# furio1999/EO_Diffusion

Hardware: AMD Instinct MI355X
Metric: denoising steps/sec (UNet fwd + DDPM update) at 256x256 bs=16 (higher is better)
Workload: dtype f32; 1 GPU; DDPM sampling step, 256x256x3, batch 16 per GPU, UNet arch A0 (base 128, mults [1,2,3,4], 1 res-block(s), attn_res []), Philox noise, x0-clipped update; global_batch=16, image_size=256, parallelism=batch-sharded x1, accumulate=fp32, precision_mode=fp32x3

## Files before the change

### eo_diffusion_amd/csrc/igemm.hip

```cpp
#include <type_traits>

#include "common.h"

struct IgemmP {
    const char* a0;
    const char* a1;
    const char* b;
    const float* bias;
    const float* cbias;
    const char* res;
    char* y;
    long long cbias_stride;
    int N, H, W, C0, C1, Cin, Cout, KS, stride, pad, ups, pad_tl, Ho, Wo, HoWo, Heff, Weff;
    int tw_log2, th;
    int tiles_pw, tiles_pi;
    long long lda, ldb, ldc, sa0, sa1, sb0, sb1, sc0, sc1;
    int nb1, bias_mode, c_f32;
    long long M;
    int Ncols, K, taps, KT, tiles_m, tiles_n, out_nchw;
    int kc0, kc1;
    int tapmajor_log2;
    int ldk;
    const float* gn_ss;
    int gn_silu;
// ... 1021 lines not shown
            const int hi = (UPS ? tg.ty0 / 2 : tg.ty0) - 1 + py, wi = (UPS ? tg.tx0 / 2 : tg.tx0) - 1 + px;
            const bool ok = (wave + NW * i) < PG && prow < PR && (unsigned)hi < (unsigned)p.H && (unsigned)wi < (unsigned)p.W;
            if (ok) pvalid |= 1u << i;
            ppix[i] = (unsigned)(hi * p.W + wi);
        }
    };
    set_tile_pieces(g);
    auto pchunk_of = [&](int i) { return (int)((pck >> (3 * i)) & 7u); };
    unsigned b_v[LB];
#pragma unroll
    for (int i = 0; i < LB; ++i) {
        const int row = (wave + NW * i) * 8 + srow;
        b_v[i] = (n0 + row < p.Ncols) ? (unsigned)(row * p.Cin * ES) + bchunk0 * 16 : EOD_OOB;
    }
    const __amdgpu_buffer_rsrc_t rsA0 = make_rsrc(p.a0 + (long long)g.n_first * p.H * p.W * p.C0 * ES);
    const __amdgpu_buffer_rsrc_t rsA1 = make_rsrc(p.a1 ? p.a1 + (long long)g.n_first * p.H * p.W * p.C1 * ES : p.a0);
    const __amdgpu_buffer_rsrc_t rsB = make_rsrc(p.b + (long long)n0 * p.Cin * ES);
    const int tapstride = p.Cout * p.Cin * ES;
    __amdgpu_buffer_rsrc_t rsS = rsB;
    if constexpr (GN)
        rsS = __builtin_amdgcn_make_buffer_rsrc(const_cast<float*>(p.gn_ss) + (long long)g.n_first * p.Cin * 2, 0, p.Cin * 8, 0x00020000);

    struct Chunk {
        int src, kin, cw;
        unsigned bk;
        bool ktail;
    };
    auto chunk_of = [&](int cc) {
        Chunk c;
        c.src = cc >= p.kc0 ? 1 : 0;
        const int ci = c.src ? cc - p.kc0 : cc;
        c.kin = ci * BK;
        c.cw = c.src ? p.C1 : p.C0;
        c.bk = (unsigned)(((c.src ? p.C0 : 0) + c.kin) * ES);
        c.ktail = c.kin + BK > c.cw;
        return c;
    };
    auto issue_patch_piece = [&](int i, const Chunk& c, char* abuf) {
        const int pc = pchunk_of(i);
        unsigned v = ((pvalid >> i) & 1u) ? ppix[i] * (unsigned)(c.cw * ES) + pc * 16 : EOD_OOB;
        if (__builtin_expect(c.ktail, 0)) v = (c.kin + pc * EPC < c.cw) ? v : EOD_OOB;
        if (c.src)
            blds16(rsA1, v, (unsigned)(c.kin * ES), abuf + (wave + NW * i) * 1024);
        else
            blds16(rsA0, v, (unsigned)(c.kin * ES), abuf + (wave + NW * i) * 1024);
    };
    auto issue_ss = [&](const Chunk& c, char* ssbuf) {
        const unsigned v = lane < 32 ? (unsigned)(lane * 16 + ((c.src ? p.C0 : 0) + c.kin) * 8) : EOD_OOB;
        __builtin_amdgcn_raw_ptr_buffer_load_lds(rsS, (lds_void*)ssbuf, 16, v, 0, 0, 0);
    };
    struct XfPre {
        i32x4 raw;
        f32x4 q[GN ? (ES == 2 ? 4 : 2) : 1];
    };
    auto xf_load = [&](int i, char* abuf, const char* ssbuf, XfPre& pre) {
        const int pc = pchunk_of(i);
        pre.raw = *reinterpret_cast<const i32x4*>(abuf + (wave + NW * i) * 1024 + lane * 16);
        if constexpr (GN) {
            const float* sp = reinterpret_cast<const float*>(ssbuf) + pc * EPC * 2;
#pragma unroll
            for (int k = 0; k < (ES == 2 ? 4 : 2); ++k) pre.q[k] = *reinterpret_cast<const f32x4*>(sp + 4 * k);
        }
    };
    auto xf_finish = [&](int i, const Chunk& c, char* abuf, const XfPre& pre) {
        const int pc = pchunk_of(i);
        const bool ok = ((pvalid >> i) & 1u) && (!c.ktail || (c.kin + pc * EPC < c.cw));
        char* ptr = abuf + (wave + NW * i) * 1024 + lane * 16;
        const i32x4 raw = pre.raw;
        i32x4 outv = raw;
        if constexpr (GN) {
            if constexpr (ES == 2) {
                const half8 h = __builtin_bit_cast(half8, raw);
                half8 o;
#pragma unroll
                for (int e = 0; e < 8; ++e) {
                    float v = (float)h[e] * pre.q[e >> 1][(e & 1) * 2] + pre.q[e >> 1][(e & 1) * 2 + 1];
                    v = v * __builtin_amdgcn_rcpf(1.0f + __builtin_amdgcn_exp2f(__builtin_fmaf(v, silu_k, silu_c)));
                    o[e] = (half_t)v;
                }
                outv = __builtin_bit_cast(i32x4, o);
            } else {
                const f32x4 f = __builtin_bit_cast(f32x4, raw);
                f32x4 o;
                const f32x4 q0 = pre.q[0], q1 = pre.q[GN && ES != 2 ? 1 : 0];
                const float sc[4] = {q0[0], q0[2], q1[0], q1[2]}, sh[4] = {q0[1], q0[3], q1[1], q1[3]};
#pragma unroll
                for (int e = 0; e < 4; ++e) {
                    float v = f[e] * sc[e] + sh[e];
                    if constexpr (SPLIT) {
                        v = v * __builtin_amdgcn_rcpf(1.0f + __builtin_amdgcn_exp2f(__builtin_fmaf(v, silu_k, silu_c)));
                    } else {
                        if (p.gn_silu) v = silu_f<SPLIT>(v);
                    }
                    o[e] = v;
                }
                outv = __builtin_bit_cast(i32x4, o);
            }
            if constexpr (!SPLIT) {
                if (!ok) outv = raw;
            }
        }
        if constexpr (SPLIT) {
            const float sl = (GN && !ok) ? 0.0f : asc.s;
            *reinterpret_cast<i32x4*>(ptr) = split_pair_exchange_scaled(__builtin_bit_cast(f32x4, outv), sl, (pc & 1) != 0);
        } else {
            if (ok) *reinterpret_cast<i32x4*>(ptr) = outv;
        }
    };
    auto transform_piece = [&](int i, const Chunk& c, char* abuf, const char* ssbuf) {
        XfPre pre;
        xf_load(i, abuf, ssbuf, pre);
        xf_finish(i, c, abuf, pre);
    };
    unsigned bve[LB];
    auto weight_offsets = [&](const Chunk& c, unsigned (&out)[LB]) {
        const bool kok = !c.ktail || (c.kin + (SPLIT ? (bchunk0 >> 1) * 8 : bchunk0 * EPC) < c.cw);
#pragma unroll
        for (int i = 0; i < LB; ++i) out[i] = kok ? b_v[i] : EOD_OOB;
    };
    auto issue_weights_at = [&](int tap, const Chunk& c, const unsigned (&off)[LB], char* bst) {
        const unsigned soff = (unsigned)(tap * tapstride) + c.bk;
#pragma unroll
        for (int i = 0; i < LB; ++i) blds16(rsB, off[i], soff, bst + (wave + NW * i) * 1024);
    };
    auto issue_weights = [&](int tap, const Chunk& c, char* bst) {
        unsigned off[LB];
        weight_offsets(c, off);
        issue_weights_at(tap, c, off, bst);
    };

    typename AccLayout<MS>::vec acc[TM][TN];
#pragma unroll
    for (int i = 0; i < TM; ++i)
#pragma unroll
        for (int j = 0; j < TN; ++j)
#pragma unroll
            for (int r = 0; r < AccLayout<MS>::R; ++r) acc[i][j][r] = 0.0f;

    const int lr = lane & (MS - 1), lh = MS == 32 ? lane >> 5 : lane >> 4;
    int prow0[TM], pyo[TM], pxo[TM];
#pragma unroll
    for (int i = 0; i < TM; ++i) {
        const int r = wm * WM + i * MS + lr;
        pyo[i] = r >> 4;
        pxo[i] = r & 15;
        prow0[i] = pyo[i] * PW + pxo[i];
    }
    const int bsw = (lr >> 1) & 7;
    int bcoff[4];
#pragma unroll
    for (int s = 0; s < 4; ++s) bcoff[s] = ((2 * s + lh) ^ bsw) * 16;
    const int b_rd = (wn * WN + lr) * BKB;
    int acur[2][3] = {{0, 0, 0}, {0, 0, 0}};
    auto aimm = [](int i, int dy) { return (UPS ? ((i + dy + 1) >> 1) : (i + dy)) * PW * BKB; };
    if constexpr (MS == 16) {
        constexpr int LROW = WM / 16;
        static_assert(LROW % 2 == 0, "the UPS row split needs an even first tile row per wave");
        const int c0 = SPLIT ? 2 * ((0x2130 >> (4 * lh)) & 3) : lh, c1 = SPLIT ? c0 + 1 : 4 + lh;
#pragma unroll
        for (int dx = 0; dx < 3; ++dx) {
            const int pxc = UPS ? ((lr + dx + 1) >> 1) : lr + dx;
            const int key = (pxc >> 1) & 7;
            const int rowb = ((UPS ? (wm * LROW) >> 1 : wm * LROW) * PW + pxc) * BKB;
            acur[0][dx] = rowb + ((c0 ^ key) << 4);
            acur[1][dx] = rowb + ((c1 ^ key) << 4);
        }
    }

    const int KC = p.kc0 + p.kc1;
    int kc_begin = 0, kc_end = KC;
    if constexpr (KSPLIT) {
        kc_begin = (int)blockIdx.y * p.splitk_per;
        kc_end = (int)blockIdx.y == p.splitk - 1 ? KC : kc_begin + p.splitk_per;
    }
    const int NSTEP = (kc_end - kc_begin) * 9;
    const int TSTEP = NSTEP * ntile;
    {
        const Chunk c0 = chunk_of(kc_begin);
#pragma unroll
        for (int i = 0; i < LAH; ++i)
            if ((wave + NW * i) < PG) issue_patch_piece(i, c0, sA);
        if constexpr (GN) {
            if (wave == 0) issue_ss(c0, sS);
        }
        issue_weights(0, c0, sB);
        if constexpr (XF) {
            asm volatile("s_waitcnt vmcnt(0)" ::: "memory");
            if constexpr (GN) __builtin_amdgcn_s_barrier();
#pragma unroll
            for (int i = 0; i < LAH; ++i)
                if ((wave + NW * i) < PG) transform_piece(i, c0, sA, sS);
            __builtin_amdgcn_s_waitcnt(0xc07f);
        }
    }
    EOD_STAMP_AT(1);
    int pp1 = 0;
    int step = 0;
    int qpar = 0;
    for (int k = 0; k < ntile; ++k) {
    for (int cc = kc_begin; cc < kc_end; ++cc) {
        const Chunk cur = chunk_of(cc);
        const bool next_tile = STREAM && cc + 1 == kc_end && k + 1 < ntile;
        const bool has_next = cc + 1 < kc_end || next_tile;
        const Chunk nxt = chunk_of(cc + 1 < kc_end ? cc + 1 : (next_tile ? 0 : cc));
        if constexpr (STREAM) {
            if (next_tile) set_tile_pieces(make_geom<true, BM>(p, tile_m + k + 1));
        }
        const char* abuf = sA + qpar * ABUF;
        char* abuf_next = sA + (qpar ^ 1) * ABUF;
        weight_offsets(cur, bve);
#pragma unroll
        for (int t = 0; t < 9; ++t, ++step) {
            EOD_TSTAMP_AT(4 * t + 0);
            if (!(STREAM && t == 0 && cc == kc_begin && k > 0)) {
                if (pp1 == 0) asm volatile("s_waitcnt vmcnt(0)" ::: "memory");
                else if (pp1 == 1) asm volatile("s_waitcnt vmcnt(1)" ::: "memory");
                else asm volatile("s_waitcnt vmcnt(2)" ::: "memory");
                if constexpr (XF) __builtin_amdgcn_s_waitcnt(0xc07f);
                __builtin_amdgcn_s_barrier();
            }
            EOD_TSTAMP_AT(4 * t + 1);
            if (step + 1 < TSTEP) {
                if (t < 8) issue_weights_at(t + 1, cur, bve, sB + ((step + 1) & 1) * BSTAGE);
                else issue_weights(0, nxt, sB + ((step + 1) & 1) * BSTAGE);
            }
            pp1 = 0;
            if (t < LAH && has_next && (wave + NW * t) < PG) {
                issue_patch_piece(t, nxt, abuf_next);
                pp1 = 1;
            }
            if constexpr (GN) {
                if (t == 0 && has_next && wave == 0) {
                    issue_ss(nxt, sS + (qpar ^ 1) * 1024);
                    ++pp1;
                }
            }
            EOD_TSTAMP_AT(4 * t + 2);
            const int dy = t / 3, dx = t - dy * 3;
            const char* bst = sB + (step & 1) * BSTAGE;
            int arow[TM], asw[TM];
#pragma unroll
            for (int i = 0; i < TM; ++i) {
                const int pxc = UPS ? ((pxo[i] + dx + 1) >> 1) : pxo[i] + dx;
                const int prow = UPS ? ((pyo[i] + dy + 1) >> 1) * PW + pxc : prow0[i] + dy * PW + dx;
                arow[i] = prow * BKB;
                asw[i] = (pxc >> 1) & 7;
            }
            if constexpr (MS == 16 && SPLIT) {
                const int ch = 2 * ((0x2130 >> (4 * lh)) & 3);
                i32x4 ah[TM], al[TM], bh[TN], bl[TN];
#pragma unroll
                for (int i = 0; i < TM; ++i) al[i] = *reinterpret_cast<const i32x4*>(sA + acur[1][dx] + aimm(i, dy));
#pragma unroll
                for (int j = 0; j < TN; ++j) bh[j] = *reinterpret_cast<const i32x4*>(bst + b_rd + j * MS * BKB + ((ch ^ bsw) << 4));
#pragma unroll
                for (int i = 0; i < TM; ++i) ah[i] = *reinterpret_cast<const i32x4*>(sA + acur[0][dx] + aimm(i, dy));
#pragma unroll
                for (int i = 0; i < TM; ++i)
#pragma unroll
                    for (int j = 0; j < TN; ++j)
                        acc[i][j] = DIRECT ? __builtin_amdgcn_mfma_f32_16x16x32_f16(__builtin_bit_cast(half8, bh[j]), __builtin_bit_cast(half8, al[i]), acc[i][j], 0, 0, 0)
                                           : __builtin_amdgcn_mfma_f32_16x16x32_f16(__builtin_bit_cast(half8, al[i]), __builtin_bit_cast(half8, bh[j]), acc[i][j], 0, 0, 0);
#pragma unroll
                for (int j = 0; j < TN; ++j) bl[j] = *reinterpret_cast<const i32x4*>(bst + b_rd + j * MS * BKB + (((ch + 1) ^ bsw) << 4));
#pragma unroll
                for (int i = 0; i < TM; ++i)
#pragma unroll
                    for (int j = 0; j < TN; ++j)
                        acc[i][j] = DIRECT ? __builtin_amdgcn_mfma_f32_16x16x32_f16(__builtin_bit_cast(half8, bl[j]), __builtin_bit_cast(half8, ah[i]), acc[i][j], 0, 0, 0)
                                           : __builtin_amdgcn_mfma_f32_16x16x32_f16(__builtin_bit_cast(half8, ah[i]), __builtin_bit_cast(half8, bl[j]), acc[i][j], 0, 0, 0);
#pragma unroll
                for (int i = 0; i < TM; ++i)
#pragma unroll
                    for (int j = 0; j < TN; ++j)
                        acc[i][j] = DIRECT ? __builtin_amdgcn_mfma_f32_16x16x32_f16(__builtin_bit_cast(half8, bh[j]), __builtin_bit_cast(half8, ah[i]), acc[i][j], 0, 0, 0)
                                           : __builtin_amdgcn_mfma_f32_16x16x32_f16(__builtin_bit_cast(half8, ah[i]), __builtin_bit_cast(half8, bh[j]), acc[i][j], 0, 0, 0);
            } else if constexpr (MS == 16) {
#pragma unroll
                for (int s = 0; s < 2; ++s) {
                    const int ch = 4 * s + lh;
                    i32x4 fa16[TM], fb16[TN];
#pragma unroll
                    for (int i = 0; i < TM; ++i) fa16[i] = *reinterpret_cast<const i32x4*>(sA + acur[s][dx] + aimm(i, dy));
#pragma unroll
                    for (int j = 0; j < TN; ++j) fb16[j] = *reinterpret_cast<const i32x4*>(bst + b_rd + j * MS * BKB + ((ch ^ bsw) << 4));
#pragma unroll
                    for (int i = 0; i < TM; ++i)
#pragma unroll
                        for (int j = 0; j < TN; ++j)
                            acc[i][j] = __builtin_amdgcn_mfma_f32_16x16x32_f16(__builtin_bit_cast(half8, fa16[i]), __builtin_bit_cast(half8, fb16[j]), acc[i][j], 0, 0, 0);
                }
            } else {
            i32x4 fa[2][TM], fb[2][TN];
#pragma unroll
            for (int i = 0; i < TM; ++i)
                fa[0][i] = *reinterpret_cast<const i32x4*>(abuf + arow[i] + (((0 + lh) ^ asw[i]) << 4));
#pragma unroll
            for (int j = 0; j < TN; ++j) fb[0][j] = *reinterpret_cast<const i32x4*>(bst + b_rd + j * 32 * BKB + bcoff[0]);
            __builtin_amdgcn_sched_group_barrier(0x100, TM + TN, 0);
#pragma unroll
            for (int s = 0; s < 4; ++s) {
                const int cur = s & 1, nx = cur ^ 1;
                if (s < 3) {
#pragma unroll
                    for (int i = 0; i < TM; ++i)
                        fa[nx][i] = *reinterpret_cast<const i32x4*>(abuf + arow[i] + (((2 * (s + 1) + lh) ^ asw[i]) << 4));
#pragma unroll
                    for (int j = 0; j < TN; ++j)
                        fb[nx][j] = *reinterpret_cast<const i32x4*>(bst + b_rd + j * 32 * BKB + bcoff[s + 1]);
                    __builtin_amdgcn_sched_group_barrier(0x100, TM + TN, 0);
                }
#pragma unroll
                for (int i = 0; i < TM; ++i)
#pragma unroll
                    for (int j = 0; j < TN; ++j) Mma<T>::run(fa[cur][i], fb[cur][j], acc[i][j]);
                __builtin_amdgcn_sched_group_barrier(0x008, TM * TN * (sizeof(T) == 4 ? 4 : 1), 0);
            }
            }
            EOD_TSTAMP_AT(4 * t + 3);
            if constexpr (XF) {
                if (t >= 2 && t - 2 < LAH && has_next && (wave + NW * (t - 2)) < PG)
                    transform_piece(t - 2, nxt, abuf_next, sS + (qpar ^ 1) * 1024);
            }
        }
        EOD_TSTAMP_AT(36);
#ifdef EOD_TSTAMP
        if (GN && wave == 1 && cc == 1 && k == 0 && blockIdx.x < 2048) {
            __builtin_amdgcn_s_waitcnt(0xc07f);
            if (lane < 37) g_eod_tstamp[blockIdx.x][lane] = reinterpret_cast<const unsigned long long*>(sA + ABUF + PR * 128)[lane];
        }
#endif
        if constexpr (MS == 16) {
            const int flip = qpar ? -ABUF : ABUF;
#pragma unroll
            for (int dx = 0; dx < 3; ++dx) {
                acur[0][dx] += flip;
                acur[1][dx] += flip;
            }
        }
        qpar ^= 1;
    }
    if constexpr (SKIP) {
      if (!KSPLIT || (int)blockIdx.y == p.splitk - 1) {
        constexpr int LA = BM / 8 / NW;
        constexpr int STG_A = BM * BKB, STG = STG_A + BSTAGE;
        static_assert(2 * STG <= 2 * ABUF + BSTAGES * BSTAGE, "the skip phase reuses the operand ring");
        __builtin_amdgcn_s_waitcnt(0xc07f);
        __builtin_amdgcn_s_barrier();
        const int SC = p.SC0 + p.SC1;
        const __amdgpu_buffer_rsrc_t rsX0 = make_rsrc(p.sx0 + (long long)g.n_first * p.H * p.W * p.SC0 * ES);
        const __amdgpu_buffer_rsrc_t rsX1 = make_rsrc(p.sx1 ? p.sx1 + (long long)g.n_first * p.H * p.W * p.SC1 * ES : p.sx0);
        const __amdgpu_buffer_rsrc_t rsW2 = make_rsrc(p.b2 + (long long)n0 * SC * ES);
        unsigned xpix[LA], wv[LB];
        unsigned xok = 0;
#pragma unroll
        for (int i = 0; i < LA; ++i) {
            const int row = (wave + NW * i) * 8 + srow;
            xpix[i] = (unsigned)((g.ty0 + (row >> 4)) * p.W + g.tx0 + (row & 15));
            if (g.tx0 + (row & 15) < p.W) xok |= 1u << i;
        }
#pragma unroll
        for (int i = 0; i < LB; ++i) {
            const int row = (wave + NW * i) * 8 + srow;
            wv[i] = (n0 + row < p.Ncols) ? (unsigned)(row * SC * ES) + bchunk0 * 16 : EOD_OOB;
        }
        auto issue_skip = [&](int kt, char* stg) {
            const int src = kt >= p.skc0 ? 1 : 0;
            const int kin = (src ? kt - p.skc0 : kt) * BK, cw = src ? p.SC1 : p.SC0;
            const bool ktail = kin + BK > cw;
#pragma unroll
            for (int i = 0; i < LA; ++i) {
                unsigned v = ((xok >> i) & 1u) ? xpix[i] * (unsigned)(cw * ES) + bchunk0 * 16 : EOD_OOB;
                if (ktail) v = (kin + bchunk0 * EPC < cw) ? v : EOD_OOB;
                if (src)
                    blds16(rsX1, v, (unsigned)(kin * ES), stg + (wave + NW * i) * 1024);
                else
                    blds16(rsX0, v, (unsigned)(kin * ES), stg + (wave + NW * i) * 1024);
            }
#pragma unroll
            for (int i = 0; i < LB; ++i) {
                unsigned v = wv[i];
                if (ktail) v = (kin + (SPLIT ? (bchunk0 >> 1) * 8 : bchunk0 * EPC) < cw) ? v : EOD_OOB;
                blds16(rsW2, v, (unsigned)(((src ? p.SC0 : 0) + kin) * ES), stg + STG_A + (wave + NW * i) * 1024);
            }
        };
        const int KS = p.skc0 + p.skc1;
        const int a_rd = (wm * WM + lr) * BKB;
        const int b_rd2 = STG_A + (wn * WN + lr) * BKB;
        if (KS > 0) issue_skip(0, smem);
        for (int kt = 0; kt < KS; ++kt) {
            char* stg = smem + (kt & 1) * STG;
            asm volatile("s_waitcnt vmcnt(0)" ::: "memory");
            if constexpr (SPLIT) {
#pragma unroll
                for (int i = 0; i < LA; ++i) {
                    char* ptr = stg + (wave + NW * i) * 1024 + lane * 16;
                    const f32x4 f = *reinterpret_cast<const f32x4*>(ptr);
                    *reinterpret_cast<i32x4*>(ptr) = split_pair_exchange_scaled(f, asc.s, (bchunk0 & 1) != 0);
                }
                __builtin_amdgcn_s_waitcnt(0xc07f);
            }
            __builtin_amdgcn_s_barrier();
            if (kt + 1 < KS) issue_skip(kt + 1, smem + ((kt + 1) & 1) * STG);
            if constexpr (SPLIT) {
                const int ch = 2 * ((0x2130 >> (4 * lh)) & 3);
                const int ohi = (ch ^ bsw) * 16, olo = ((ch + 1) ^ bsw) * 16;
                i32x4 ah[TM], al[TM], bh[TN], bl[TN];
#pragma unroll
                for (int i = 0; i < TM; ++i) al[i] = *reinterpret_cast<const i32x4*>(stg + a_rd + i * MS * BKB + olo);
#pragma unroll
                for (int j = 0; j < TN; ++j) bh[j] = *reinterpret_cast<const i32x4*>(stg + b_rd2 + j * MS * BKB + ohi);
#pragma unroll
                for (int i = 0; i < TM; ++i) ah[i] = *reinterpret_cast<const i32x4*>(stg + a_rd + i * MS * BKB + ohi);
#pragma unroll
                for (int i = 0; i < TM; ++i)
#pragma unroll
                    for (int j = 0; j < TN; ++j)
                        acc[i][j] = DIRECT ? __builtin_amdgcn_mfma_f32_16x16x32_f16(__builtin_bit_cast(half8, bh[j]), __builtin_bit_cast(half8, al[i]), acc[i][j], 0, 0, 0)
                                           : __builtin_amdgcn_mfma_f32_16x16x32_f16(__builtin_bit_cast(half8, al[i]), __builtin_bit_cast(half8, bh[j]), acc[i][j], 0, 0, 0);
#pragma unroll
                for (int j = 0; j < TN; ++j) bl[j] = *reinterpret_cast<const i32x4*>(stg + b_rd2 + j * MS * BKB + olo);
#pragma unroll
                for (int i = 0; i < TM; ++i)
#pragma unroll
                    for (int j = 0; j < TN; ++j)
                        acc[i][j] = DIRECT ? __builtin_amdgcn_mfma_f32_16x16x32_f16(__builtin_bit_cast(half8, bl[j]), __builtin_bit_cast(half8, ah[i]), acc[i][j], 0, 0, 0)
                                           : __builtin_amdgcn_mfma_f32_16x16x32_f16(__builtin_bit_cast(half8, ah[i]), __builtin_bit_cast(half8, bl[j]), acc[i][j], 0, 0, 0);
#pragma unroll
                for (int i = 0; i < TM; ++i)
#pragma unroll
                    for (int j = 0; j < TN; ++j)
                        acc[i][j] = DIRECT ? __builtin_amdgcn_mfma_f32_16x16x32_f16(__builtin_bit_cast(half8, bh[j]), __builtin_bit_cast(half8, ah[i]), acc[i][j], 0, 0, 0)
                                           : __builtin_amdgcn_mfma_f32_16x16x32_f16(__builtin_bit_cast(half8, ah[i]), __builtin_bit_cast(half8, bh[j]), acc[i][j], 0, 0, 0);
            } else {
#pragma unroll
                for (int s2 = 0; s2 < 2; ++s2) {
                    const int o = ((4 * s2 + lh) ^ bsw) * 16;
                    i32x4 fa16[TM], fb16[TN];
#pragma unroll
                    for (int i = 0; i < TM; ++i) fa16[i] = *reinterpret_cast<const i32x4*>(stg + a_rd + i * MS * BKB + o);
#pragma unroll
                    for (int j = 0; j < TN; ++j) fb16[j] = *reinterpret_cast<const i32x4*>(stg + b_rd2 + j * MS * BKB + o);
#pragma unroll
                    for (int i = 0; i < TM; ++i)
#pragma unroll
                        for (int j = 0; j < TN; ++j)
                            acc[i][j] = __builtin_amdgcn_mfma_f32_16x16x32_f16(__builtin_bit_cast(half8, fa16[i]), __builtin_bit_cast(half8, fb16[j]), acc[i][j], 0, 0, 0);
                }
            }
        }
      }
    }
    if constexpr (STREAM) {
        if (k + 1 < ntile) {
            asm volatile("s_waitcnt vmcnt(0)" ::: "memory");
            __builtin_amdgcn_s_waitcnt(0xc07f);
            __builtin_amdgcn_s_barrier();
        }
    } else {
        __builtin_amdgcn_s_waitcnt(0xc07f);
        __builtin_amdgcn_s_barrier();
    }
    EOD_STAMP_AT(2);
    IgemmP pe = p;
    if constexpr (KSPLIT) pe.y = p.y + (long long)blockIdx.y * p.M * p.Cout * 4;
    if constexpr (SPLIT) {
        pe.alpha = p.alpha * wsc1 * asc.inv;
        if constexpr (DIRECT) halo_epilogue_direct<BM, BN, WAVES_M, WAVES_N>(pe, g, acc, wave, lane, n0, pre_bq, pe.alpha, pre_we);
        else igemm_epilogue<T, true, BM, BN, WAVES_M, WAVES_N, true, MS>(pe, g, acc, smem, wave, lane, n0, nullptr, 0, pre_bcol);
    } else if constexpr (sizeof(T) == 2) {
        igemm_epilogue<T, true, BM, BN, WAVES_M, WAVES_N, KSPLIT, MS>(pe, g, acc, smem, wave, lane, n0, nullptr, 0, pre_bcol);
    } else {
        igemm_epilogue<T, true, BM, BN, WAVES_M, WAVES_N, sizeof(T) == 4, MS>(pe, g, acc, smem, wave, lane, n0, nullptr, 0, pre_bcol);
    }
    if constexpr (STREAM) {
        if (k + 1 < ntile) {
            g = make_geom<true, BM>(p, tile_m + k + 1);
#pragma unroll
            for (int i = 0; i < TM; ++i)
#pragma unroll
                for (int j = 0; j < TN; ++j)
#pragma unroll
                    for (int r = 0; r < AccLayout<MS>::R; ++r) acc[i][j][r] = 0.0f;
        }
    }
    }
    EOD_STAMP_AT(3);
}

template <typename T, bool SPLIT, bool BWD = false>
__global__ __launch_bounds__(256, 2) void conv_up4_halo_kernel(const IgemmP p) {
    static_assert(!SPLIT || sizeof(T) == 4, "the split-fp16 product is a mode of fp32 storage");
    static_assert(SPLIT || sizeof(T) == 2, "fp16 storage or split fp32");
    constexpr int NW = 4, WAVES_M = 2, WAVES_N = 2, BN = 128, BM = 128, MS = 16;
    constexpr int PH = 10, PW = 18, PR = PH * PW, PG = (PR + 7) / 8, LAH = (PG + NW - 1) / NW;
    constexpr int ES = sizeof(T), EPC = 16 / ES, BKB = 128, BK = BKB / ES;
    constexpr int WM = BM / WAVES_M, WN = BN / WAVES_N, TM = WM / MS, TN = WN / MS;
    constexpr int LB = (BN / 8) / NW;
    constexpr int ABUF = PG * 1024, BSTAGE = BN * BKB;
    static_assert(LAH == 6, "schedule: three patch pieces per K-step in steps 0 and 1");

    extern __shared__ __attribute__((aligned(16))) char smem[];
    char* const sA = smem;
    char* const sB = smem + 2 * ABUF;

    constexpr bool DIRECT = SPLIT && !BWD;
    const int tid = threadIdx.x, lane = tid & 63;
    const int wave = __builtin_amdgcn_readfirstlane(tid >> 6);
    const int wm = wave / WAVES_N, wn = wave % WAVES_N;
    int tile_m, tile_nn;
    map_tile(p, tile_m, tile_nn);
    const int tpc = BWD ? p.tiles_n : p.tiles_n >> 2;
    const int cls = BWD ? 0 : tile_nn / tpc, n0 = (tile_nn - cls * tpc) * BN;
    const int par_y = cls >> 1, par_x = cls & 1;
    const TileGeom g = make_geom<true, BM>(p, tile_m);
    float pre_bcol[DIRECT ? 1 : TN];
    f32x4 pre_bq[DIRECT ? TN : 1];
    int pre_we[DIRECT ? TN : 1];
    if constexpr (DIRECT) {
        prefetch_bcol4<TN>(p, p.Cout, n0 + wn * WN, lane, g.n_first, pre_bq);
        prefetch_wexp4<TN>(p, p.Cout, n0 + wn * WN, cls * p.Cout, lane, pre_we);
    } else {
        prefetch_bcol<TN, MS>(p, p.Cout, n0 + wn * WN, lane, g.n_first, pre_bcol);
    }
    float wsc1 = 1.0f;
    if constexpr (SPLIT) wsc1 = p.w_scale[1];
    AbScale asc = {EOD_SPLIT_ASCALE, 1.0f};
    if constexpr (SPLIT) {
        if (p.a_bound) asc = ab_scale_of(ab_wave_bound(p.a_bound, g.n_first));
    }

    const int srow = lane >> 3, sslot = lane & 7;
    unsigned ppix[LAH];
    const int bchunk0 = sslot ^ ((4 * wave + (srow >> 1)) & 7);
    unsigned pck = 0, pvalid = 0;
#pragma unroll
    for (int i = 0; i < LAH; ++i) {
        const int prow = (wave + NW * i) * 8 + srow;
        const int py = prow / PW, px = prow - py * PW;
        const int hi = g.ty0 - 1 + py, wi = g.tx0 - 1 + px;
        const bool ok = (wave + NW * i) < PG && prow < PR && (unsigned)hi < (unsigned)p.H && (unsigned)wi < (unsigned)p.W;
        if (ok) pvalid |= 1u << i;
        ppix[i] = BWD ? (unsigned)(4 * hi * p.W + 2 * wi)
                      : (unsigned)(hi * p.W + wi);
        pck |= (unsigned)(sslot ^ ((px >> 1) & 7)) << (3 * i);
    }
    auto pchunk_of = [&](int i) { return (int)((pck >> (3 * i)) & 7u); };
    unsigned b_v[LB];
#pragma unroll
    for (int i = 0; i < LB; ++i) {
        const int row = (wave + NW * i) * 8 + srow;
        b_v[i] = (n0 + row < p.Cout) ? (unsigned)(row * (BWD ? 4 * p.C0 : p.Cin) * ES) + bchunk0 * 16 : EOD_OOB;
    }
    const __amdgpu_buffer_rsrc_t rsA = make_rsrc(p.a0 + (long long)g.n_first * p.H * p.W * p.C0 * ES * (BWD ? 4 : 1));
    const int bpitch = BWD ? 4 * p.C0 : p.Cin;
    const __amdgpu_buffer_rsrc_t rsB = make_rsrc(p.b + ((long long)cls * p.Cout + n0) * bpitch * ES);
    const int tapstride = (BWD ? p.Cout * bpitch : 4 * p.Cout * p.Cin) * ES;

    struct Chunk {
        int kin, cls;
        bool ktail;
    };
    auto chunk_of = [&](int cc) {
        Chunk c;
        c.cls = BWD ? (cc & 3) : cls;
        c.kin = (BWD ? (cc >> 2) : cc) * BK;
        c.ktail = c.kin + BK > p.C0;
        return c;
    };
    auto issue_patch_piece = [&](int i, const Chunk& c, char* abuf) {
        const int pc = pchunk_of(i);
        unsigned v = ((pvalid >> i) & 1u) ? ppix[i] * (unsigned)(p.C0 * ES) + pc * 16 : EOD_OOB;
        if (c.ktail) v = (c.kin + pc * EPC < p.C0) ? v : EOD_OOB;
        const unsigned soff = (unsigned)(c.kin * ES) + (BWD ? (unsigned)(((c.cls >> 1) * 2 * p.W + (c.cls & 1)) * p.C0 * ES) : 0u);
        blds16(rsA, v, soff, abuf + (wave + NW * i) * 1024);
    };
    auto split_piece = [&](int i, char* abuf) {
        char* ptr = abuf + (wave + NW * i) * 1024 + lane * 16;
        const f32x4 f = *reinterpret_cast<const f32x4*>(ptr);
        *reinterpret_cast<i32x4*>(ptr) = split_pair_exchange_scaled(f, asc.s, (pchunk_of(i) & 1) != 0);
    };
    auto issue_weights = [&](int s, const Chunk& c, char* bst) {
        const int oy = BWD ? 1 - (c.cls >> 1) : par_y, ox = BWD ? 1 - (c.cls & 1) : par_x;
        const int tap = (oy + (s >> 1)) * 3 + ox + (s & 1);
        const unsigned soff = (unsigned)(tap * tapstride) + (unsigned)((c.kin + (BWD ? c.cls * p.C0 : 0)) * ES);
#pragma unroll
        for (int i = 0; i < LB; ++i) {
            unsigned v = b_v[i];
            if (c.ktail) v = (c.kin + (SPLIT ? (bchunk0 >> 1) * 8 : bchunk0 * EPC) < p.C0) ? v : EOD_OOB;
            blds16(rsB, v, soff, bst + (wave + NW * i) * 1024);
        }
    };
    auto wait_vm = [](int n) {
        switch (n) {
            case 0: asm volatile("s_waitcnt vmcnt(0)" ::: "memory"); break;
            case 1: asm volatile("s_waitcnt vmcnt(1)" ::: "memory"); break;
            case 2: asm volatile("s_waitcnt vmcnt(2)" ::: "memory"); break;
            case 3: asm volatile("s_waitcnt vmcnt(3)" ::: "memory"); break;
            case 4: asm volatile("s_waitcnt vmcnt(4)" ::: "memory"); break;
            case 5: asm volatile("s_waitcnt vmcnt(5)" ::: "memory"); break;
            default: asm volatile("s_waitcnt vmcnt(6)" ::: "memory"); break;
        }
    };

    typename AccLayout<MS>::vec acc[TM][TN];
#pragma unroll
    for (int i = 0; i < TM; ++i)
#pragma unroll
        for (int j = 0; j < TN; ++j)
#pragma unroll
            for (int r = 0; r < AccLayout<MS>::R; ++r) acc[i][j][r] = 0.0f;

    const int lr = lane & 15, lh = lane >> 4;
    const int c0 = SPLIT ? 2 * ((0x2130 >> (4 * lh)) & 3) : lh, c1 = SPLIT ? c0 + 1 : 4 + lh;
    int acur[2][2];
    auto set_acur = [&](int oy, int ox, int aoff) {
#pragma unroll
        for (int b = 0; b < 2; ++b) {
            const int pxc = lr + ox + b;
            const int key = (pxc >> 1) & 7;
            const int rowb = ((wm * (WM / 16) + oy) * PW + pxc) * BKB + aoff;
            acur[0][b] = rowb + ((c0 ^ key) << 4);
            acur[1][b] = rowb + ((c1 ^ key) << 4);
        }
    };
    set_acur(BWD ? 1 : par_y, BWD ? 1 : par_x, 0);
    const int bsw = (lr >> 1) & 7;
    const int b_rd = (wn * WN + lr) * BKB;
    const int boff0 = b_rd + ((c0 ^ bsw) << 4), boff1 = b_rd + ((c1 ^ bsw) << 4);

    const int KC = BWD ? 4 * p.kc0 : p.kc0, NSTEP = KC * 4;
    {
        const Chunk ch0 = chunk_of(0);
#pragma unroll
        for (int i = 0; i < LAH; ++i)
            if ((wave + NW * i) < PG) issue_patch_piece(i, ch0, sA);
        issue_weights(0, ch0, sB);
        if constexpr (SPLIT) {
            asm volatile("s_waitcnt vmcnt(0)" ::: "memory");
#pragma unroll
            for (int i = 0; i < LAH; ++i)
                if ((wave + NW * i) < PG) split_piece(i, sA);
        }
    }
    int np_prev = 0;
    int step = 0;
    for (int cc = 0; cc < KC; ++cc) {
        const Chunk cur = chunk_of(cc);
        const bool has_next = cc + 1 < KC;
        const Chunk nxt = chunk_of(has_next ? cc + 1 : cc);
        char* abuf_next = sA + ((cc + 1) & 1) * ABUF;
#pragma unroll
        for (int s = 0; s < 4; ++s, ++step) {
            wait_vm(np_prev);
            if constexpr (SPLIT) __builtin_amdgcn_s_waitcnt(0xc07f);
            __builtin_amdgcn_s_barrier();
            const bool w_next = step + 1 < NSTEP;
            if (w_next) issue_weights((s + 1) & 3, s == 3 ? nxt : cur, sB + ((step + 1) & 1) * BSTAGE);
            int np = 0;
            if (s < 2 && has_next) {
#pragma unroll
                for (int k = 0; k < 3; ++k)
                    if ((wave + NW * (3 * s + k)) < PG) {
                        issue_patch_piece(3 * s + k, nxt, abuf_next);
                        ++np;
                    }
            }
            const int a = s >> 1, b = s & 1;
            const char* bst = sB + (step & 1) * BSTAGE;
            if constexpr (SPLIT) {
                i32x4 ah[TM], al[TM], bh[TN], bl[TN];
#pragma unroll
                for (int i = 0; i < TM; ++i) al[i] = *reinterpret_cast<const i32x4*>(sA + acur[1][b] + (i + a) * PW * BKB);
#pragma unroll
                for (int j = 0; j < TN; ++j) bh[j] = *reinterpret_cast<const i32x4*>(bst + boff0 + j * MS * BKB);
#pragma unroll
                for (int i = 0; i < TM; ++i) ah[i] = *reinterpret_cast<const i32x4*>(sA + acur[0][b] + (i + a) * PW * BKB);
#pragma unroll
                for (int i = 0; i < TM; ++i)
#pragma unroll
                    for (int j = 0; j < TN; ++j)
                        acc[i][j] = DIRECT ? __builtin_amdgcn_mfma_f32_16x16x32_f16(__builtin_bit_cast(half8, bh[j]), __builtin_bit_cast(half8, al[i]), acc[i][j], 0, 0, 0)
                                           : __builtin_amdgcn_mfma_f32_16x16x32_f16(__builtin_bit_cast(half8, al[i]), __builtin_bit_cast(half8, bh[j]), acc[i][j], 0, 0, 0);
#pragma unroll
                for (int j = 0; j < TN; ++j) bl[j] = *reinterpret_cast<const i32x4*>(bst + boff1 + j * MS * BKB);
#pragma unroll
                for (int i = 0; i < TM; ++i)
#pragma unroll
                    for (int j = 0; j < TN; ++j)
                        acc[i][j] = DIRECT ? __builtin_amdgcn_mfma_f32_16x16x32_f16(__builtin_bit_cast(half8, bl[j]), __builtin_bit_cast(half8, ah[i]), acc[i][j], 0, 0, 0)
                                           : __builtin_amdgcn_mfma_f32_16x16x32_f16(__builtin_bit_cast(half8, ah[i]), __builtin_bit_cast(half8, bl[j]), acc[i][j], 0, 0, 0);
#pragma unroll
                for (int i = 0; i < TM; ++i)
#pragma unroll
                    for (int j = 0; j < TN; ++j)
                        acc[i][j] = DIRECT ? __builtin_amdgcn_mfma_f32_16x16x32_f16(__builtin_bit_cast(half8, bh[j]), __builtin_bit_cast(half8, ah[i]), acc[i][j], 0, 0, 0)
                                           : __builtin_amdgcn_mfma_f32_16x16x32_f16(__builtin_bit_cast(half8, ah[i]), __builtin_bit_cast(half8, bh[j]), acc[i][j], 0, 0, 0);
            } else {
#pragma unroll
                for (int v = 0; v < 2; ++v) {
                    i32x4 fa16[TM], fb16[TN];
#pragma unroll
                    for (int i = 0; i < TM; ++i) fa16[i] = *reinterpret_cast<const i32x4*>(sA + acur[v][b] + (i + a) * PW * BKB);
#pragma unroll
                    for (int j = 0; j < TN; ++j) fb16[j] = *reinterpret_cast<const i32x4*>(bst + (v ? boff1 : boff0) + j * MS * BKB);
#pragma unroll
                    for (int i = 0; i < TM; ++i)
#pragma unroll
                        for (int j = 0; j < TN; ++j)
                            acc[i][j] = __builtin_amdgcn_mfma_f32_16x16x32_f16(__builtin_bit_cast(half8, fa16[i]), __builtin_bit_cast(half8, fb16[j]), acc[i][j], 0, 0, 0);
                }
            }
            if constexpr (SPLIT) {
                if (s >= 2 && has_next) {
#pragma unroll
                    for (int k = 0; k < 3; ++k)
                        if ((wave + NW * (3 * (s - 2) + k)) < PG) split_piece(3 * (s - 2) + k, abuf_next);
                }
            }
            np_prev = np;
        }
        if constexpr (BWD) {
            const int ncl = (cc + 1) & 3;
            set_acur(1 - (ncl >> 1), 1 - (ncl & 1), ((cc + 1) & 1) * ABUF);
        } else {
            const int flip = (cc & 1) ? -ABUF : ABUF;
#pragma unroll
            for (int b = 0; b < 2; ++b) {
                acur[0][b] += flip;
                acur[1][b] += flip;
            }
        }
    }
    __builtin_amdgcn_s_waitcnt(0xc07f);
    __builtin_amdgcn_s_barrier();
    IgemmP pe = p;
    pe.Ncols = p.Cout;
    TileGeom ge = g;
    if constexpr (!BWD) {
        pe.par = 1; pe.par_y = par_y; pe.par_x = par_x;
        pe.Wd = p.W;
        pe.tiles_per_image = p.tiles_pi * 4;
        ge.tile_m = g.n_first * pe.tiles_per_image + (tile_m - g.n_first * p.tiles_pi) * 4 + cls;
    }
    if constexpr (SPLIT) pe.alpha = p.alpha * wsc1 * asc.inv;
    if constexpr (!BWD) pe.w_row0 = cls * p.Cout;
    if constexpr (DIRECT) halo_epilogue_direct<BM, BN, WAVES_M, WAVES_N>(pe, ge, acc, wave, lane, n0, pre_bq, pe.alpha, pre_we);
    else igemm_epilogue<T, true, BM, BN, WAVES_M, WAVES_N, sizeof(T) == 4, MS>(pe, ge, acc, smem, wave, lane, n0, nullptr, 0, pre_bcol);
}

template <typename T, bool SPLIT, bool BWD = false> static int launch_up4(IgemmP& p, hipStream_t st) {
    constexpr int BK = 128 / (int)sizeof(T);
    const size_t ring = 2 * (size_t)(23 * 1024) + 2 * (size_t)128 * 128;
    const size_t epi = 4 * (size_t)64 * (64 + 4) * sizeof(float);
    const size_t lds = ring > epi ? ring : epi;
    auto kern = conv_up4_halo_kernel<T, SPLIT, BWD>;
    static bool attr_done = false;
    if (!attr_done) {
        (void)hipFuncSetAttribute(reinterpret_cast<const void*>(kern), hipFuncAttributeMaxDynamicSharedMemorySize, (int)lds);
        attr_done = true;
    }
    p.kc0 = (p.C0 + BK - 1) / BK;
    p.kc1 = 0;
    p.KT = p.kc0 * 4;
    p.tiles_n = (BWD ? 1 : 4) * ((p.Cout + 127) / 128);
    p.tw_log2 = 4;
    p.th = 8;
    p.tiles_pw = (p.W + 15) / 16;
    p.tiles_pi = p.tiles_pw * (p.H / 8);
    p.tiles_m = p.tiles_pi * p.N;
    const long long nblk = (long long)p.tiles_m * p.tiles_n;
    if (nblk <= 0 || nblk > 0x7fffffffLL) {
        eod_set_error("conv_up4: bad grid %lld", nblk);
        return EOD_EINVAL;
    }
    hipLaunchKernelGGL(kern, dim3((unsigned)nblk), dim3(256), lds, st, p);
    EOD_CHECK_LAUNCH("conv_up4_halo");
    return EOD_OK;
}

template <typename T, bool SPLIT>
__global__ __launch_bounds__(256, 2) void conv_s2_halo_kernel(const IgemmP p) {
    static_assert(!SPLIT || sizeof(T) == 4, "the split-fp16 product is a mode of fp32 storage");
    static_assert(SPLIT || sizeof(T) == 2, "fp16 storage or split fp32");
    constexpr int NW = 4, WAVES_M = 2, WAVES_N = 2, BN = 128, BM = 128, MS = 16;
    constexpr int PH = 9, PW = 17, PR = PH * PW, PG = (PR + 7) / 8, LAH = (PG + NW - 1) / NW;
    constexpr int ES = sizeof(T), EPC = 16 / ES, BKB = 128, BK = BKB / ES;
    constexpr int WM = BM / WAVES_M, WN = BN / WAVES_N, TM = WM / MS, TN = WN / MS;
    constexpr int LB = (BN / 8) / NW;
    constexpr int ABUF = PG * 1024, BSTAGE = BN * BKB;
    static_assert(PG == NW * LAH && LAH * 4 <= 32, "every wave stages LAH whole pieces; 4 plane-validity bits per piece");
    static_assert(LB <= 6, "wait_vm immediates");

    extern __shared__ __attribute__((aligned(16))) char smem[];
    char* const sA = smem;
    char* const sB = smem + 2 * ABUF;

    constexpr bool DIRECT = SPLIT;
    const int tid = threadIdx.x, lane = tid & 63;
    const int wave = __builtin_amdgcn_readfirstlane(tid >> 6);
    const int wm = wave / WAVES_N, wn = wave % WAVES_N;
    int tile_m, tile_n;
    map_tile(p, tile_m, tile_n);
    const int n0 = tile_n * BN;
    const TileGeom g = make_geom<true, BM>(p, tile_m);
    float pre_bcol[DIRECT ? 1 : TN];
    f32x4 pre_bq[DIRECT ? TN : 1];
    int pre_we[DIRECT ? TN : 1];
    if constexpr (DIRECT) {
        prefetch_bcol4<TN>(p, p.Cout, n0 + wn * WN, lane, g.n_first, pre_bq);
        prefetch_wexp4<TN>(p, p.Cout, n0 + wn * WN, 0, lane, pre_we);
    } else {
        prefetch_bcol<TN, MS>(p, p.Cout, n0 + wn * WN, lane, g.n_first, pre_bcol);
    }
    float wsc1 = 1.0f;
    if constexpr (SPLIT) wsc1 = p.w_scale[1];
    AbScale asc = {EOD_SPLIT_ASCALE, 1.0f};
    if constexpr (SPLIT) {
        if (p.a_bound) asc = ab_scale_of(ab_wave_bound(p.a_bound, g.n_first));
    }

    const int srow = lane >> 3, sslot = lane & 7;
    int ppix[LAH];
    unsigned pvalid = 0, pck = 0;
    const int bchunk0 = sslot ^ ((4 * wave + (srow >> 1)) & 7);
#pragma unroll
    for (int i = 0; i < LAH; ++i) {
        const int prow = (wave + NW * i) * 8 + srow;
        const int py = prow / PW, px = prow - py * PW;
        const int hi = 2 * (g.ty0 + py) - 1, wi = 2 * (g.tx0 + px) - 1;
        ppix[i] = hi * p.W + wi;
#pragma unroll
        for (int pl = 0; pl < 4; ++pl) {
            const bool ok = prow < PR && (unsigned)(hi + (pl >> 1)) < (unsigned)p.H && (unsigned)(wi + (pl & 1)) < (unsigned)p.W;
            if (ok) pvalid |= 1u << (4 * i + pl);
        }
        pck |= (unsigned)(sslot ^ ((px >> 1) & 7)) << (3 * i);
    }
    auto pchunk_of = [&](int i) { return (int)((pck >> (3 * i)) & 7u); };
    unsigned b_v[LB];
#pragma unroll
    for (int i = 0; i < LB; ++i) {
        const int row = (wave + NW * i) * 8 + srow;
        b_v[i] = (n0 + row < p.Cout) ? (unsigned)(row * p.Cin * ES) + bchunk0 * 16 : EOD_OOB;
    }
    const __amdgpu_buffer_rsrc_t rsA = make_rsrc(p.a0 + (long long)g.n_first * p.H * p.W * p.C0 * ES);
    const __amdgpu_buffer_rsrc_t rsB = make_rsrc(p.b + (long long)n0 * p.Cin * ES);
    const int tapstride = p.Cout * p.Cin * ES;

    auto issue_patch_piece = [&](int i, int kin, int pl, char* abuf) {
        const int pc = pchunk_of(i);
        unsigned v = ((pvalid >> (4 * i + pl)) & 1u) ? (unsigned)(ppix[i] + (pl >> 1) * p.W + (pl & 1)) * (unsigned)(p.C0 * ES) + pc * 16 : EOD_OOB;
        if (kin + BK > p.C0) v = (kin + pc * EPC < p.C0) ? v : EOD_OOB;
        blds16(rsA, v, (unsigned)(kin * ES), abuf + (wave + NW * i) * 1024);
    };
    auto split_piece = [&](int i, char* abuf) {
        char* ptr = abuf + (wave + NW * i) * 1024 + lane * 16;
        const f32x4 f = *reinterpret_cast<const f32x4*>(ptr);
        *reinterpret_cast<i32x4*>(ptr) = split_pair_exchange_scaled(f, asc.s, (pchunk_of(i) & 1) != 0);
    };
    auto issue_weights = [&](int tap, int kin, char* bst) {
        const unsigned soff = (unsigned)(tap * tapstride) + (unsigned)(kin * ES);
#pragma unroll
// ... 1297 lines not shown
```

Measured before the change: 38.94 steps/s.

## Reorder conv taps dy-inner and reuse A-fragment rows in a register window

```diff
diff --git a/eo_diffusion_amd/csrc/igemm.hip b/eo_diffusion_amd/csrc/igemm.hip
--- a/eo_diffusion_amd/csrc/igemm.hip
+++ b/eo_diffusion_amd/csrc/igemm.hip
@@ -1197,7 +1197,16 @@
     for (int s = 0; s < 4; ++s) bcoff[s] = ((2 * s + lh) ^ bsw) * 16;
     const int b_rd = (wn * WN + lr) * BKB;
     int acur[2][3] = {{0, 0, 0}, {0, 0, 0}};
-    auto aimm = [](int i, int dy) { return (UPS ? ((i + dy + 1) >> 1) : (i + dy)) * PW * BKB; };
+    auto aoff = [](int r) { return (UPS ? ((r + 1) >> 1) : r) * PW * BKB; };
+    i32x4 aw[2][TM];
+    constexpr bool WINDOW = !STREAM;
+    auto a_load = [&](int v, int dx, int dy) {
+#pragma unroll
+        for (int r = 0; r < TM + 2; ++r)
+            if (dy == 0 || !WINDOW ? (r >= dy && r < TM + dy) : r == TM - 1 + dy) aw[v][r % TM] = *reinterpret_cast<const i32x4*>(sA + acur[v][dx] + aoff(r));
+    };
+    constexpr bool EARLY = WINDOW && MS == 16 && WAVES_N == 4;
+    auto tap_slot = [](int t) { return MS == 16 ? 3 * (t % 3) + t / 3 : t; };
     if constexpr (MS == 16) {
         constexpr int LROW = WM / 16;
         static_assert(LROW % 2 == 0, "the UPS row split needs an even first tile row per wave");
@@ -1266,7 +1275,7 @@
             }
             EOD_TSTAMP_AT(4 * t + 1);
             if (step + 1 < TSTEP) {
-                if (t < 8) issue_weights_at(t + 1, cur, bve, sB + ((step + 1) & 1) * BSTAGE);
+                if (t < 8) issue_weights_at(tap_slot(t + 1), cur, bve, sB + ((step + 1) & 1) * BSTAGE);
                 else issue_weights(0, nxt, sB + ((step + 1) & 1) * BSTAGE);
             }
             pp1 = 0;
@@ -1281,7 +1290,9 @@
                 }
             }
             EOD_TSTAMP_AT(4 * t + 2);
-            const int dy = t / 3, dx = t - dy * 3;
+            const int dy = MS == 16 ? t % 3 : t / 3, dx = MS == 16 ? t / 3 : t % 3;
+            const int ndy = (t + 1) % 3, ndx = (t + 1) / 3;
+            const bool a_here = !EARLY || t == 0, a_early = EARLY && t < 8;
             const char* bst = sB + (step & 1) * BSTAGE;
             int arow[TM], asw[TM];
 #pragma unroll
@@ -1293,47 +1304,47 @@
             }
             if constexpr (MS == 16 && SPLIT) {
                 const int ch = 2 * ((0x2130 >> (4 * lh)) & 3);
-                i32x4 ah[TM], al[TM], bh[TN], bl[TN];
-#pragma unroll
-                for (int i = 0; i < TM; ++i) al[i] = *reinterpret_cast<const i32x4*>(sA + acur[1][dx] + aimm(i, dy));
+                i32x4 bh[TN], bl[TN];
+                if (a_here) a_load(1, dx, dy);
 #pragma unroll
                 for (int j = 0; j < TN; ++j) bh[j] = *reinterpret_cast<const i32x4*>(bst + b_rd + j * MS * BKB + ((ch ^ bsw) << 4));
-#pragma unroll
-                for (int i = 0; i < TM; ++i) ah[i] = *reinterpret_cast<const i32x4*>(sA + acur[0][dx] + aimm(i, dy));
+                if (a_here) a_load(0, dx, dy);
 #pragma unroll
                 for (int i = 0; i < TM; ++i)
 #pragma unroll
                     for (int j = 0; j < TN; ++j)
-                        acc[i][j] = DIRECT ? __builtin_amdgcn_mfma_f32_16x16x32_f16(__builtin_bit_cast(half8, bh[j]), __builtin_bit_cast(half8, al[i]), acc[i][j], 0, 0, 0)
-                                           : __builtin_amdgcn_mfma_f32_16x16x32_f16(__builtin_bit_cast(half8, al[i]), __builtin_bit_cast(half8, bh[j]), acc[i][j], 0, 0, 0);
+                        acc[i][j] = DIRECT ? __builtin_amdgcn_mfma_f32_16x16x32_f16(__builtin_bit_cast(half8, bh[j]), __builtin_bit_cast(half8, aw[1][(i + dy) % TM]), acc[i][j], 0, 0, 0)
+                                           : __builtin_amdgcn_mfma_f32_16x16x32_f16(__builtin_bit_cast(half8, aw[1][(i + dy) % TM]), __builtin_bit_cast(half8, bh[j]), acc[i][j], 0, 0, 0);
 #pragma unroll
                 for (int j = 0; j < TN; ++j) bl[j] = *reinterpret_cast<const i32x4*>(bst + b_rd + j * MS * BKB + (((ch + 1) ^ bsw) << 4));
+                if (a_early) a_load(1, ndx, ndy);
 #pragma unroll
                 for (int i = 0; i < TM; ++i)
 #pragma unroll
                     for (int j = 0; j < TN; ++j)
-                        acc[i][j] = DIRECT ? __builtin_amdgcn_mfma_f32_16x16x32_f16(__builtin_bit_cast(half8, bl[j]), __builtin_bit_cast(half8, ah[i]), acc[i][j], 0, 0, 0)
-                                           : __builtin_amdgcn_mfma_f32_16x16x32_f16(__builtin_bit_cast(half8, ah[i]), __builtin_bit_cast(half8, bl[j]), acc[i][j], 0, 0, 0);
+                        acc[i][j] = DIRECT ? __builtin_amdgcn_mfma_f32_16x16x32_f16(__builtin_bit_cast(half8, bl[j]), __builtin_bit_cast(half8, aw[0][(i + dy) % TM]), acc[i][j], 0, 0, 0)
+                                           : __builtin_amdgcn_mfma_f32_16x16x32_f16(__builtin_bit_cast(half8, aw[0][(i + dy) % TM]), __builtin_bit_cast(half8, bl[j]), acc[i][j], 0, 0, 0);
 #pragma unroll
                 for (int i = 0; i < TM; ++i)
 #pragma unroll
                     for (int j = 0; j < TN; ++j)
-                        acc[i][j] = DIRECT ? __builtin_amdgcn_mfma_f32_16x16x32_f16(__builtin_bit_cast(half8, bh[j]), __builtin_bit_cast(half8, ah[i]), acc[i][j], 0, 0, 0)
-                                           : __builtin_amdgcn_mfma_f32_16x16x32_f16(__builtin_bit_cast(half8, ah[i]), __builtin_bit_cast(half8, bh[j]), acc[i][j], 0, 0, 0);
+                        acc[i][j] = DIRECT ? __builtin_amdgcn_mfma_f32_16x16x32_f16(__builtin_bit_cast(half8, bh[j]), __builtin_bit_cast(half8, aw[0][(i + dy) % TM]), acc[i][j], 0, 0, 0)
+                                           : __builtin_amdgcn_mfma_f32_16x16x32_f16(__builtin_bit_cast(half8, aw[0][(i + dy) % TM]), __builtin_bit_cast(half8, bh[j]), acc[i][j], 0, 0, 0);
+                if (a_early) a_load(0, ndx, ndy);
             } else if constexpr (MS == 16) {
 #pragma unroll
                 for (int s = 0; s < 2; ++s) {
                     const int ch = 4 * s + lh;
-                    i32x4 fa16[TM], fb16[TN];
-#pragma unroll
-                    for (int i = 0; i < TM; ++i) fa16[i] = *reinterpret_cast<const i32x4*>(sA + acur[s][dx] + aimm(i, dy));
+                    i32x4 fb16[TN];
+                    if (a_here) a_load(s, dx, dy);
 #pragma unroll
                     for (int j = 0; j < TN; ++j) fb16[j] = *reinterpret_cast<const i32x4*>(bst + b_rd + j * MS * BKB + ((ch ^ bsw) << 4));
 #pragma unroll
                     for (int i = 0; i < TM; ++i)
 #pragma unroll
                         for (int j = 0; j < TN; ++j)
-                            acc[i][j] = __builtin_amdgcn_mfma_f32_16x16x32_f16(__builtin_bit_cast(half8, fa16[i]), __builtin_bit_cast(half8, fb16[j]), acc[i][j], 0, 0, 0);
+                            acc[i][j] = __builtin_amdgcn_mfma_f32_16x16x32_f16(__builtin_bit_cast(half8, aw[s][(i + dy) % TM]), __builtin_bit_cast(half8, fb16[j]), acc[i][j], 0, 0, 0);
+                    if (a_early) a_load(s, ndx, ndy);
                 }
             } else {
             i32x4 fa[2][TM], fb[2][TN];
@@ -1627,7 +1638,7 @@
     };
     auto issue_weights = [&](int s, const Chunk& c, char* bst) {
         const int oy = BWD ? 1 - (c.cls >> 1) : par_y, ox = BWD ? 1 - (c.cls & 1) : par_x;
-        const int tap = (oy + (s >> 1)) * 3 + ox + (s & 1);
+        const int tap = (oy + (s & 1)) * 3 + ox + (s >> 1);
         const unsigned soff = (unsigned)(tap * tapstride) + (unsigned)((c.kin + (BWD ? c.cls * p.C0 : 0)) * ES);
 #pragma unroll
         for (int i = 0; i < LB; ++i) {
@@ -1674,6 +1685,12 @@
     const int b_rd = (wn * WN + lr) * BKB;
     const int boff0 = b_rd + ((c0 ^ bsw) << 4), boff1 = b_rd + ((c1 ^ bsw) << 4);
 
+    i32x4 aw[2][TM];
+    auto a_load = [&](int v, int b, int a) {
+#pragma unroll
+        for (int r = 0; r < TM + 1; ++r)
+            if (a == 0 ? r < TM : r == TM) aw[v][r % TM] = *reinterpret_cast<const i32x4*>(sA + acur[v][b] + r * PW * BKB);
+    };
     const int KC = BWD ? 4 * p.kc0 : p.kc0, NSTEP = KC * 4;
     {
         const Chunk ch0 = chunk_of(0);
@@ -1711,49 +1728,46 @@
                         ++np;
                     }
             }
-            const int a = s >> 1, b = s & 1;
+            const int a = s & 1, b = s >> 1;
             const char* bst = sB + (step & 1) * BSTAGE;
             if constexpr (SPLIT) {
-                i32x4 ah[TM], al[TM], bh[TN], bl[TN];
-#pragma unroll
-                for (int i = 0; i < TM; ++i) al[i] = *reinterpret_cast<const i32x4*>(sA + acur[1][b] + (i + a) * PW * BKB);
+                i32x4 bh[TN], bl[TN];
+                a_load(1, b, a);
 #pragma unroll
                 for (int j = 0; j < TN; ++j) bh[j] = *reinterpret_cast<const i32x4*>(bst + boff0 + j * MS * BKB);
-#pragma unroll
-                for (int i = 0; i < TM; ++i) ah[i] = *reinterpret_cast<const i32x4*>(sA + acur[0][b] + (i + a) * PW * BKB);
+                a_load(0, b, a);
 #pragma unroll
                 for (int i = 0; i < TM; ++i)
 #pragma unroll
                     for (int j = 0; j < TN; ++j)
-                        acc[i][j] = DIRECT ? __builtin_amdgcn_mfma_f32_16x16x32_f16(__builtin_bit_cast(half8, bh[j]), __builtin_bit_cast(half8, al[i]), acc[i][j], 0, 0, 0)
-                                           : __builtin_amdgcn_mfma_f32_16x16x32_f16(__builtin_bit_cast(half8, al[i]), __builtin_bit_cast(half8, bh[j]), acc[i][j], 0, 0, 0);
+                        acc[i][j] = DIRECT ? __builtin_amdgcn_mfma_f32_16x16x32_f16(__builtin_bit_cast(half8, bh[j]), __builtin_bit_cast(half8, aw[1][(i + a) % TM]), acc[i][j], 0, 0, 0)
+                                           : __builtin_amdgcn_mfma_f32_16x16x32_f16(__builtin_bit_cast(half8, aw[1][(i + a) % TM]), __builtin_bit_cast(half8, bh[j]), acc[i][j], 0, 0, 0);
 #pragma unroll
                 for (int j = 0; j < TN; ++j) bl[j] = *reinterpret_cast<const i32x4*>(bst + boff1 + j * MS * BKB);
 #pragma unroll
                 for (int i = 0; i < TM; ++i)
 #pragma unroll
                     for (int j = 0; j < TN; ++j)
-                        acc[i][j] = DIRECT ? __builtin_amdgcn_mfma_f32_16x16x32_f16(__builtin_bit_cast(half8, bl[j]), __builtin_bit_cast(half8, ah[i]), acc[i][j], 0, 0, 0)
-                                           : __builtin_amdgcn_mfma_f32_16x16x32_f16(__builtin_bit_cast(half8, ah[i]), __builtin_bit_cast(half8, bl[j]), acc[i][j], 0, 0, 0);
+                        acc[i][j] = DIRECT ? __builtin_amdgcn_mfma_f32_16x16x32_f16(__builtin_bit_cast(half8, bl[j]), __builtin_bit_cast(half8, aw[0][(i + a) % TM]), acc[i][j], 0, 0, 0)
+                                           : __builtin_amdgcn_mfma_f32_16x16x32_f16(__builtin_bit_cast(half8, aw[0][(i + a) % TM]), __builtin_bit_cast(half8, bl[j]), acc[i][j], 0, 0, 0);
 #pragma unroll
                 for (int i = 0; i < TM; ++i)
 #pragma unroll
                     for (int j = 0; j < TN; ++j)
-                        acc[i][j] = DIRECT ? __builtin_amdgcn_mfma_f32_16x16x32_f16(__builtin_bit_cast(half8, bh[j]), __builtin_bit_cast(half8, ah[i]), acc[i][j], 0, 0, 0)
-                                           : __builtin_amdgcn_mfma_f32_16x16x32_f16(__builtin_bit_cast(half8, ah[i]), __builtin_bit_cast(half8, bh[j]), acc[i][j], 0, 0, 0);
+                        acc[i][j] = DIRECT ? __builtin_amdgcn_mfma_f32_16x16x32_f16(__builtin_bit_cast(half8, bh[j]), __builtin_bit_cast(half8, aw[0][(i + a) % TM]), acc[i][j], 0, 0, 0)
+                                           : __builtin_amdgcn_mfma_f32_16x16x32_f16(__builtin_bit_cast(half8, aw[0][(i + a) % TM]), __builtin_bit_cast(half8, bh[j]), acc[i][j], 0, 0, 0);
             } else {
 #pragma unroll
                 for (int v = 0; v < 2; ++v) {
-                    i32x4 fa16[TM], fb16[TN];
-#pragma unroll
-                    for (int i = 0; i < TM; ++i) fa16[i] = *reinterpret_cast<const i32x4*>(sA + acur[v][b] + (i + a) * PW * BKB);
+                    i32x4 fb16[TN];
+                    a_load(v, b, a);
 #pragma unroll
                     for (int j = 0; j < TN; ++j) fb16[j] = *reinterpret_cast<const i32x4*>(bst + (v ? boff1 : boff0) + j * MS * BKB);
 #pragma unroll
                     for (int i = 0; i < TM; ++i)
 #pragma unroll
                         for (int j = 0; j < TN; ++j)
-                            acc[i][j] = __builtin_amdgcn_mfma_f32_16x16x32_f16(__builtin_bit_cast(half8, fa16[i]), __builtin_bit_cast(half8, fb16[j]), acc[i][j], 0, 0, 0);
+                            acc[i][j] = __builtin_amdgcn_mfma_f32_16x16x32_f16(__builtin_bit_cast(half8, aw[v][(i + a) % TM]), __builtin_bit_cast(half8, fb16[j]), acc[i][j], 0, 0, 0);
                 }
             }
             if constexpr (SPLIT) {
```

Result: faster. 40.23 steps/s (median of 6 runs) (+3.3%).
